# Hawkeye-FineGrained/Hawkeye

Hardware: NVIDIA H100
Metric: 448x448 images/sec, BCNN VGG-16 train step (fwd+CE+bwd+grad all-reduce+SGD), device-timed, max over ranks (higher is better)
Workload: dtype tf32 (fp32 storage, fp32 accumulate)

## Files before the change

### hawkeye_b200/csrc/common.cuh

```cuda
#pragma once
#include <cuda.h>
#include <cuda_runtime.h>
#include <stdint.h>
#include <stdio.h>

namespace hk {

#ifndef HK_SPIN_LIMIT
#define HK_SPIN_LIMIT (1u << 26)
#endif

__device__ __forceinline__ uint32_t smem_u32(const void* p) {
  return static_cast<uint32_t>(__cvta_generic_to_shared(p));
}

__device__ __forceinline__ void mbar_init(uint64_t* bar, uint32_t count) {
  asm volatile("mbarrier.init.shared::cta.b64 [%0], %1;" ::"r"(smem_u32(bar)), "r"(count));
}
__device__ __forceinline__ void fence_barrier_init() {
  asm volatile("fence.mbarrier_init.release.cluster;" ::: "memory");
}
__device__ __forceinline__ void fence_proxy_async() {
  asm volatile("fence.proxy.async.shared::cta;" ::: "memory");
}
__device__ __forceinline__ void mbar_expect_tx(uint64_t* bar, uint32_t bytes) {
  asm volatile("mbarrier.arrive.expect_tx.shared::cta.b64 _, [%0], %1;" ::"r"(smem_u32(bar)), "r"(bytes)
               : "memory");
}
__device__ __forceinline__ void mbar_arrive(uint64_t* bar) {
  asm volatile("mbarrier.arrive.shared::cta.b64 _, [%0];" ::"r"(smem_u32(bar)) : "memory");
}
__device__ __forceinline__ bool mbar_try_wait(uint64_t* bar, uint32_t parity) {
  uint32_t ok;
  asm volatile(
      "{\n"
      ".reg .pred p;\n"
      "mbarrier.try_wait.parity.shared::cta.b64 p, [%1], %2;\n"
      "selp.u32 %0, 1, 0, p;\n"
      "}\n"
      : "=r"(ok)
      : "r"(smem_u32(bar)), "r"(parity)
      : "memory");
  return ok != 0;
}
__device__ __forceinline__ void mbar_wait(uint64_t* bar, uint32_t parity) {
  uint32_t spins = 0;
  while (!mbar_try_wait(bar, parity)) {
    if (++spins > HK_SPIN_LIMIT) __trap();
  }
}
__device__ __forceinline__ void mbar_wait_unguarded(uint64_t* bar, uint32_t parity) {
  while (!mbar_try_wait(bar, parity)) {
  }
}

template <int N>
__device__ __forceinline__ void regs_dealloc() { asm volatile("setmaxnreg.dec.sync.aligned.u32 %0;" ::"n"(N)); }
template <int N>
__device__ __forceinline__ void regs_alloc() { asm volatile("setmaxnreg.inc.sync.aligned.u32 %0;" ::"n"(N)); }

__device__ __forceinline__ void tma_prefetch_desc(const CUtensorMap* m) {
  asm volatile("prefetch.tensormap [%0];" ::"l"(m) : "memory");
}
__device__ __forceinline__ void tma_load_2d(void* dst, const CUtensorMap* m, uint64_t* bar, int c0, int c1) {
  asm volatile(
      "cp.async.bulk.tensor.2d.shared::cluster.global.mbarrier::complete_tx::bytes [%0], [%1, {%3, %4}], [%2];" ::"r"(
          smem_u32(dst)),
      "l"(m), "r"(smem_u32(bar)), "r"(c0), "r"(c1)
      : "memory");
}
__device__ __forceinline__ void tma_load_3d(void* dst, const CUtensorMap* m, uint64_t* bar, int c0, int c1, int c2) {
  asm volatile(
      "cp.async.bulk.tensor.3d.shared::cluster.global.mbarrier::complete_tx::bytes [%0], [%1, {%3, %4, %5}], [%2];" ::
          "r"(smem_u32(dst)),
      "l"(m), "r"(smem_u32(bar)), "r"(c0), "r"(c1), "r"(c2)
      : "memory");
}
__device__ __forceinline__ void tma_load_4d(void* dst, const CUtensorMap* m, uint64_t* bar, int c0, int c1, int c2,
                                            int c3) {
  asm volatile(
      "cp.async.bulk.tensor.4d.shared::cluster.global.mbarrier::complete_tx::bytes [%0], [%1, {%3, %4, %5, %6}], "
      "[%2];" ::"r"(smem_u32(dst)),
      "l"(m), "r"(smem_u32(bar)), "r"(c0), "r"(c1), "r"(c2), "r"(c3)
      : "memory");
}

__device__ __forceinline__ void wgmma_fence() { asm volatile("wgmma.fence.sync.aligned;" ::: "memory"); }
__device__ __forceinline__ void wgmma_commit() { asm volatile("wgmma.commit_group.sync.aligned;" ::: "memory"); }
template <int N>
__device__ __forceinline__ void wgmma_wait() { asm volatile("wgmma.wait_group.sync.aligned %0;" ::"n"(N) : "memory"); }
template <int NACC>
__device__ __forceinline__ void wgmma_keep(float (&d)[NACC]) {
#pragma unroll
  for (int i = 0; i < NACC; ++i) asm volatile("" : "+f"(d[i])::"memory");
}
__device__ __forceinline__ void wgmma_tf32(float (&d)[8], uint64_t adesc, uint64_t bdesc, int scale_d) {
  asm volatile(
      "{\n"
      ".reg .pred p;\n"
      "setp.ne.b32 p, %10, 0;\n"
      "wgmma.mma_async.sync.aligned.m64n16k8.f32.tf32.tf32 "
      "{%0, %1, %2, %3, %4, %5, %6, %7}, %8, %9, p, 1, 1;\n"
      "}\n"
      : "+f"(d[0]), "+f"(d[1]), "+f"(d[2]), "+f"(d[3]), "+f"(d[4]), "+f"(d[5]), "+f"(d[6]), "+f"(d[7])
      : "l"(adesc), "l"(bdesc), "r"(scale_d));
}
__device__ __forceinline__ void wgmma_tf32(float (&d)[16], uint64_t adesc, uint64_t bdesc, int scale_d) {
  asm volatile(
      "{\n"
      ".reg .pred p;\n"
      "setp.ne.b32 p, %18, 0;\n"
      "wgmma.mma_async.sync.aligned.m64n32k8.f32.tf32.tf32 "
      "{%0, %1, %2, %3, %4, %5, %6, %7, %8, %9, %10, %11, %12, %13, %14, %15}, %16, %17, p, 1, 1;\n"
      "}\n"
      : "+f"(d[0]), "+f"(d[1]), "+f"(d[2]), "+f"(d[3]), "+f"(d[4]), "+f"(d[5]), "+f"(d[6]), "+f"(d[7]), "+f"(d[8]), "+f"(d[9]), "+f"(d[10]), "+f"(d[11]), "+f"(d[12]), "+f"(d[13]), "+f"(d[14]), "+f"(d[15])
      : "l"(adesc), "l"(bdesc), "r"(scale_d));
}
__device__ __forceinline__ void wgmma_tf32(float (&d)[32], uint64_t adesc, uint64_t bdesc, int scale_d) {
  asm volatile(
      "{\n"
      ".reg .pred p;\n"
      "setp.ne.b32 p, %34, 0;\n"
      "wgmma.mma_async.sync.aligned.m64n64k8.f32.tf32.tf32 "
      "{%0, %1, %2, %3, %4, %5, %6, %7, %8, %9, %10, %11, %12, %13, %14, %15, %16, %17, %18, %19, %20, %21, %22, %23, %24, %25, %26, %27, %28, %29, %30, %31}, %32, %33, p, 1, 1;\n"
      "}\n"
      : "+f"(d[0]), "+f"(d[1]), "+f"(d[2]), "+f"(d[3]), "+f"(d[4]), "+f"(d[5]), "+f"(d[6]), "+f"(d[7]), "+f"(d[8]), "+f"(d[9]), "+f"(d[10]), "+f"(d[11]), "+f"(d[12]), "+f"(d[13]), "+f"(d[14]), "+f"(d[15]), "+f"(d[16]), "+f"(d[17]), "+f"(d[18]), "+f"(d[19]), "+f"(d[20]), "+f"(d[21]), "+f"(d[22]), "+f"(d[23]), "+f"(d[24]), "+f"(d[25]), "+f"(d[26]), "+f"(d[27]), "+f"(d[28]), "+f"(d[29]), "+f"(d[30]), "+f"(d[31])
      : "l"(adesc), "l"(bdesc), "r"(scale_d));
}
__device__ __forceinline__ void wgmma_tf32(float (&d)[64], uint64_t adesc, uint64_t bdesc, int scale_d) {
  asm volatile(
      "{\n"
      ".reg .pred p;\n"
      "setp.ne.b32 p, %66, 0;\n"
      "wgmma.mma_async.sync.aligned.m64n128k8.f32.tf32.tf32 "
      "{%0, %1, %2, %3, %4, %5, %6, %7, %8, %9, %10, %11, %12, %13, %14, %15, %16, %17, %18, %19, %20, %21, %22, %23, %24, %25, %26, %27, %28, %29, %30, %31, %32, %33, %34, %35, %36, %37, %38, %39, %40, %41, %42, %43, %44, %45, %46, %47, %48, %49, %50, %51, %52, %53, %54, %55, %56, %57, %58, %59, %60, %61, %62, %63}, %64, %65, p, 1, 1;\n"
      "}\n"
      : "+f"(d[0]), "+f"(d[1]), "+f"(d[2]), "+f"(d[3]), "+f"(d[4]), "+f"(d[5]), "+f"(d[6]), "+f"(d[7]), "+f"(d[8]), "+f"(d[9]), "+f"(d[10]), "+f"(d[11]), "+f"(d[12]), "+f"(d[13]), "+f"(d[14]), "+f"(d[15]), "+f"(d[16]), "+f"(d[17]), "+f"(d[18]), "+f"(d[19]), "+f"(d[20]), "+f"(d[21]), "+f"(d[22]), "+f"(d[23]), "+f"(d[24]), "+f"(d[25]), "+f"(d[26]), "+f"(d[27]), "+f"(d[28]), "+f"(d[29]), "+f"(d[30]), "+f"(d[31]), "+f"(d[32]), "+f"(d[33]), "+f"(d[34]), "+f"(d[35]), "+f"(d[36]), "+f"(d[37]), "+f"(d[38]), "+f"(d[39]), "+f"(d[40]), "+f"(d[41]), "+f"(d[42]), "+f"(d[43]), "+f"(d[44]), "+f"(d[45]), "+f"(d[46]), "+f"(d[47]), "+f"(d[48]), "+f"(d[49]), "+f"(d[50]), "+f"(d[51]), "+f"(d[52]), "+f"(d[53]), "+f"(d[54]), "+f"(d[55]), "+f"(d[56]), "+f"(d[57]), "+f"(d[58]), "+f"(d[59]), "+f"(d[60]), "+f"(d[61]), "+f"(d[62]), "+f"(d[63])
      : "l"(adesc), "l"(bdesc), "r"(scale_d));
}

__device__ __forceinline__ void wgmma_tf32(float (&d)[8], const uint32_t (&a)[4], uint64_t bdesc) {
  asm volatile(
      "wgmma.mma_async.sync.aligned.m64n16k8.f32.tf32.tf32 "
      "{%0, %1, %2, %3, %4, %5, %6, %7}, {%8, %9, %10, %11}, %12, 1, 1, 1;\n"
      : "+f"(d[0]), "+f"(d[1]), "+f"(d[2]), "+f"(d[3]), "+f"(d[4]), "+f"(d[5]), "+f"(d[6]), "+f"(d[7])
      : "r"(a[0]), "r"(a[1]), "r"(a[2]), "r"(a[3]), "l"(bdesc));
}
__device__ __forceinline__ void wgmma_tf32(float (&d)[16], const uint32_t (&a)[4], uint64_t bdesc) {
  asm volatile(
      "wgmma.mma_async.sync.aligned.m64n32k8.f32.tf32.tf32 "
      "{%0, %1, %2, %3, %4, %5, %6, %7, %8, %9, %10, %11, %12, %13, %14, %15}, {%16, %17, %18, %19}, %20, 1, 1, 1;\n"
      : "+f"(d[0]), "+f"(d[1]), "+f"(d[2]), "+f"(d[3]), "+f"(d[4]), "+f"(d[5]), "+f"(d[6]), "+f"(d[7]), "+f"(d[8]), "+f"(d[9]), "+f"(d[10]), "+f"(d[11]), "+f"(d[12]), "+f"(d[13]), "+f"(d[14]), "+f"(d[15])
      : "r"(a[0]), "r"(a[1]), "r"(a[2]), "r"(a[3]), "l"(bdesc));
}
__device__ __forceinline__ void wgmma_tf32(float (&d)[32], const uint32_t (&a)[4], uint64_t bdesc) {
  asm volatile(
      "wgmma.mma_async.sync.aligned.m64n64k8.f32.tf32.tf32 "
      "{%0, %1, %2, %3, %4, %5, %6, %7, %8, %9, %10, %11, %12, %13, %14, %15, %16, %17, %18, %19, %20, %21, %22, %23, %24, %25, %26, %27, %28, %29, %30, %31}, {%32, %33, %34, %35}, %36, 1, 1, 1;\n"
      : "+f"(d[0]), "+f"(d[1]), "+f"(d[2]), "+f"(d[3]), "+f"(d[4]), "+f"(d[5]), "+f"(d[6]), "+f"(d[7]), "+f"(d[8]), "+f"(d[9]), "+f"(d[10]), "+f"(d[11]), "+f"(d[12]), "+f"(d[13]), "+f"(d[14]), "+f"(d[15]), "+f"(d[16]), "+f"(d[17]), "+f"(d[18]), "+f"(d[19]), "+f"(d[20]), "+f"(d[21]), "+f"(d[22]), "+f"(d[23]), "+f"(d[24]), "+f"(d[25]), "+f"(d[26]), "+f"(d[27]), "+f"(d[28]), "+f"(d[29]), "+f"(d[30]), "+f"(d[31])
      : "r"(a[0]), "r"(a[1]), "r"(a[2]), "r"(a[3]), "l"(bdesc));
}

__device__ __forceinline__ void named_bar(int id, int count) {
  asm volatile("bar.sync %0, %1;" ::"r"(id), "r"(count) : "memory");
}

__device__ __forceinline__ uint64_t make_sdesc(uint32_t saddr) {
  uint64_t d = 0;
  d |= static_cast<uint64_t>((saddr >> 4) & 0x3FFFu);
  d |= static_cast<uint64_t>(1) << 16;
  d |= static_cast<uint64_t>(1024 >> 4) << 32;
  d |= static_cast<uint64_t>(1) << 62;
  return d;
}

__device__ __forceinline__ uint32_t ld_shared_u32(uint32_t saddr) {
  uint32_t v;
  asm volatile("ld.shared.b32 %0, [%1];" : "=r"(v) : "r"(saddr) : "memory");
  return v;
}
__device__ __forceinline__ void st_shared_v4(uint32_t saddr, uint32_t x, uint32_t y, uint32_t z, uint32_t w) {
  asm volatile("st.shared.v4.b32 [%0], {%1, %2, %3, %4};" ::"r"(saddr), "r"(x), "r"(y), "r"(z), "r"(w) : "memory");
}

__device__ __forceinline__ uint32_t sw128_off(int row, int k) {
  return (uint32_t)(row * 128 + ((((k >> 2) ^ (row & 7)) << 4) | ((k & 3) << 2)));
}

__device__ __forceinline__ void transpose_mn_tile(const uint8_t* src, uint8_t* dst, int rows, int t, int nthr,
                                                  int box_stride = 4096) {
// ... 23 lines not shown
```

### hawkeye_b200/csrc/conv.cu

```cuda
#include <stdlib.h>

#include "common.cuh"
#include "host.h"
#include "gemm.h"
#include "../../include/hawkeye_b200.h"

namespace hk {

__global__ void pack_weights_kernel(const float* __restrict__ W, float* __restrict__ Wf, float* __restrict__ Wd,
                                    int Cout, int Cin, int round) {
  const size_t n = (size_t)Cout * Cin * 9;
  for (size_t i = blockIdx.x * (size_t)blockDim.x + threadIdx.x; i < n; i += (size_t)gridDim.x * blockDim.x) {
    const int t = i % 9;
    const int ci = (i / 9) % Cin;
    const int co = i / ((size_t)9 * Cin);
    const float v = round ? tf32_round(W[i]) : W[i];
    if (Wf) Wf[((size_t)t * Cout + co) * Cin + ci] = v;
    if (Wd) Wd[((size_t)(8 - t) * Cin + ci) * Cout + co] = v;
  }
}
__global__ void unpack_wgrad_kernel(const float* __restrict__ dWp, float* __restrict__ dW, int Cout, int Cin, int accumulate) {
  const size_t n = (size_t)Cout * Cin * 9;
  for (size_t i = blockIdx.x * (size_t)blockDim.x + threadIdx.x; i < n; i += (size_t)gridDim.x * blockDim.x) {
    const int t = i % 9;
// ... 114 lines not shown
    if (a.no_round) {
#pragma unroll
      for (int j = 0; j < 8; ++j) dst[j] = make_float4(v[4 * j], v[4 * j + 1], v[4 * j + 2], v[4 * j + 3]);
    } else {
#pragma unroll
      for (int j = 0; j < 8; ++j)
        dst[j] = make_float4(tf32_round(v[4 * j]), tf32_round(v[4 * j + 1]), tf32_round(v[4 * j + 2]),
                             tf32_round(v[4 * j + 3]));
    }
    }
  }
  if ((POOLED || a.P) && co < a.Cout) epi_pool_store(a, v, a.TW, w, h, n, co, valid);
}

template <int BN>
__device__ __forceinline__ void conv_epilogue(const ConvArgs& a, const float (&acc)[BN / 2], float* acc_tile, int w0, int h0,
                                              int n0, int co0, int ct) {
  constexpr int NACC = BN / 2;
  const int lane = ct & 31, wg = ct >> 7, half = ct >> 7;
  const int q = (ct >> 5) & 3, wl = q;
  const int r = q * 32 + lane;
  const int wi = r % a.TW, hi = (r / a.TW) % a.TH, ni = r / (a.TW * a.TH);
  const int w = w0 + wi, h = h0 + hi, n = n0 + ni;
  const bool valid = (w < a.W) && (h < a.H) && (n < a.N);
  const size_t pix = ((size_t)n * a.H + h) * a.W + w;
#pragma unroll
  for (int cp = 0; cp < BN / 64; ++cp) {
    named_bar(1, 256);
#pragma unroll
    for (int i = 0; i < NACC / 4; ++i) {
      const int col = 8 * i + 2 * (lane & 3);
      if ((col >> 6) != cp) continue;
      float* dst = acc_tile + ((col >> 5) & 1) * (128 * 33);
      const int r0 = wg * 64 + wl * 16 + (lane >> 2);
      dst[r0 * 33 + (col & 31)] = acc[4 * i];
      dst[r0 * 33 + (col & 31) + 1] = acc[4 * i + 1];
      dst[(r0 + 8) * 33 + (col & 31)] = acc[4 * i + 2];
      dst[(r0 + 8) * 33 + (col & 31) + 1] = acc[4 * i + 3];
    }
    named_bar(1, 256);
    const int c = 2 * cp + half;
    float v[32];
    {
      const float* src = acc_tile + half * (128 * 33) + r * 33;
#pragma unroll
      for (int j = 0; j < 32; ++j) v[j] = src[j];
    }
    epi_chunk(a, v, w, h, n, pix, co0 + c * 32, valid);
  }
}

template <int BN>
__global__ void __launch_bounds__(CONV_THREADS, 1)
conv3x3_igemm_kernel(const __grid_constant__ CUtensorMap tmX, const __grid_constant__ CUtensorMap tmW, ConvArgs a) {
  using Cfg = ConvCfg<BN>;
  constexpr int NACC = BN / 2;
  extern __shared__ uint8_t smem_raw[];
  uint8_t* smem = reinterpret_cast<uint8_t*>((reinterpret_cast<uintptr_t>(smem_raw) + 1023) & ~uintptr_t(1023));
  uint8_t* sA = smem;
  uint8_t* sB = smem + Cfg::STAGES * Cfg::A_BYTES;
  uint64_t* full = reinterpret_cast<uint64_t*>(smem + Cfg::STAGES * Cfg::STAGE_BYTES);
  uint64_t* empty = full + Cfg::STAGES;
  float* acc_tile = reinterpret_cast<float*>(smem + Cfg::STAGES * Cfg::STAGE_BYTES + 256);

  const int warp = threadIdx.x >> 5;
  int t = blockIdx.x;
  const int tw = t % a.tiles_w; t /= a.tiles_w;
  const int th = t % a.tiles_h; t /= a.tiles_h;
  const int w0 = tw * a.TW, h0 = th * a.TH, n0 = t * a.TN;
  const int co0 = blockIdx.y * BN;
  const int nchunk = a.Cin / 32;
  const int nk = 9 * nchunk;

  if (threadIdx.x == 0) {
    tma_prefetch_desc(&tmX);
    tma_prefetch_desc(&tmW);
    for (int s = 0; s < Cfg::STAGES; ++s) { mbar_init(&full[s], 1); mbar_init(&empty[s], 2); }
    fence_barrier_init();
  }
  __syncthreads();

  if (warp < 4) {
    regs_dealloc<56>();
    if (threadIdx.x == 0) {
      for (int kb = 0; kb < nk; ++kb) {
        const int s = kb % Cfg::STAGES;
        const uint32_t ph = (kb / Cfg::STAGES) & 1;
        const int tap = kb / nchunk, ck = kb - tap * nchunk;
        const int kh = tap / 3, kw = tap - kh * 3;
        mbar_wait(&empty[s], ph ^ 1);
        mbar_expect_tx(&full[s], Cfg::STAGE_BYTES);
        tma_load_4d(sA + s * Cfg::A_BYTES, &tmX, &full[s], ck * 32, w0 * a.stride + kw - 1, h0 * a.stride + kh - 1, n0);
        tma_load_3d(sB + s * Cfg::B_BYTES, &tmW, &full[s], ck * 32, co0, tap);
      }
    }
  } else {
    regs_alloc<224>();
    const int ct = threadIdx.x - 128;
    const int wg = ct >> 7;
    float acc[NACC];
    for (int kb = 0; kb < nk; ++kb) {
      const int s = kb % Cfg::STAGES;
      const uint32_t ph = (kb / Cfg::STAGES) & 1;
      mbar_wait(&full[s], ph);
      const uint64_t a_base = make_sdesc(smem_u32(sA + s * Cfg::A_BYTES + wg * 64 * 128));
      const uint64_t b_base = make_sdesc(smem_u32(sB + s * Cfg::B_BYTES));
      wgmma_fence();
#pragma unroll
      for (int ks = 0; ks < 4; ++ks) wgmma_tf32(acc, a_base + ks * 2, b_base + ks * 2, (kb | ks) != 0);
      wgmma_commit();
      wgmma_wait<1>();
      wgmma_keep(acc);
      if (kb > 0 && (ct & 127) == 0) mbar_arrive(&empty[(kb - 1) % Cfg::STAGES]);
    }
    wgmma_wait<0>();
    wgmma_keep(acc);
    conv_epilogue<BN>(a, acc, acc_tile, w0, h0, n0, co0, ct);
  }
}

static void pick_tile(int W, int H, int N, int target, int* TW, int* TH, int* TN) {
  int tw = 1;
  while (tw * 2 <= 16 && W % (tw * 2) == 0 && tw * 2 <= target) tw *= 2;
  int th = 1;
  while (th * 2 * tw <= target && H % (th * 2) == 0) th *= 2;
  int tn = target / (tw * th);
  *TW = tw; *TH = th; *TN = tn;
  (void)N;
}

static int make_act_map(CUtensorMap* tm, const float* X, int N, int H, int W, int C, int TW, int TH, int TN,
                        int stride = 1) {
  uint64_t dims[4] = {(uint64_t)C, (uint64_t)W, (uint64_t)H, (uint64_t)N};
  uint64_t strides[3] = {(uint64_t)C * 4, (uint64_t)W * C * 4, (uint64_t)H * W * C * 4};
  uint32_t box[4] = {32, (uint32_t)(TW * stride), (uint32_t)(TH * stride), (uint32_t)TN};
  uint32_t estr[4] = {1, (uint32_t)stride, (uint32_t)stride, 1};
  return make_tmap(tm, X, 4, dims, strides, box, stride > 1 ? estr : nullptr);
}

template <int BN>
static int launch_conv(const CUtensorMap& tmX, const CUtensorMap& tmW, const ConvArgs& a, cudaStream_t stream) {
  using Cfg = ConvCfg<BN>;
  if (int r = allow_dynamic_smem<conv3x3_igemm_kernel<BN>>(Cfg::SMEM, BN == 64 ? "conv<64>" : "conv<128>")) return r;
  dim3 grid(a.tiles_w * a.tiles_h * a.tiles_n, (a.Cout + BN - 1) / BN);
  conv3x3_igemm_kernel<BN><<<grid, CONV_THREADS, Cfg::SMEM, stream>>>(tmX, tmW, a);
  HK_LAUNCH_CHECK("conv3x3_igemm_kernel");
  return 0;
}

constexpr int CONV_V2_THREADS = 512;

enum { EPI_MAP = 0, EPI_UNPOOL = 1, EPI_FIRST_WGRAD = 2 };
constexpr int FW_HALO = 3 * 10 * 18;
constexpr int FW_HALO_BYTES = 2 * FW_HALO * 4;
struct FirstWgradArgs {
  const float* img;
  float* part;
};

__device__ __forceinline__ void mma_m16n8k8_tf32(float (&d)[4], const uint32_t (&a)[4], uint32_t b0, uint32_t b1) {
  asm volatile("mma.sync.aligned.m16n8k8.row.col.f32.tf32.tf32.f32 {%0, %1, %2, %3}, {%4, %5, %6, %7}, {%8, %9}, "
               "{%0, %1, %2, %3};\n"
               : "+f"(d[0]), "+f"(d[1]), "+f"(d[2]), "+f"(d[3])
               : "r"(a[0]), "r"(a[1]), "r"(a[2]), "r"(a[3]), "r"(b0), "r"(b1));
}

template <int BN, bool RESIDENT>
struct ConvV2Cfg {
  static constexpr int A_BYTES = 160 * 128;
  static constexpr int B_TILE = BN * 128;
  static constexpr int STAGE_BYTES = A_BYTES + (RESIDENT ? 0 : 3 * B_TILE);
  static constexpr int STAGES = RESIDENT ? 2 : (BN == 64 ? 3 : 2);
  static constexpr int WRES_BYTES = RESIDENT ? 18 * B_TILE : 0;
  static constexpr int PIECES = STAGES == 2 && !RESIDENT ? 3 : 1;
  static constexpr int STG_LD = BN + 8;
  static constexpr int STG_BYTES = 128 * STG_LD * 4;
  static constexpr int SMEM = STAGES * STAGE_BYTES + WRES_BYTES + 1024 + 256 + STG_BYTES;
};

template <int BN, bool RESIDENT, int TW, int EPI>
__global__ void __launch_bounds__(CONV_V2_THREADS, 1)
conv3x3_igemm_v2_kernel(const __grid_constant__ CUtensorMap tmX, const __grid_constant__ CUtensorMap tmW, ConvArgs a,
                        int n_ntiles, int total_tiles, FirstWgradArgs fw) {
  using Cfg = ConvV2Cfg<BN, RESIDENT>;
  static_assert(EPI != EPI_FIRST_WGRAD || (BN == 64 && RESIDENT && TW == 16), "conv1_1 weight gradient: 64 -> 64, 16 x 8");
  constexpr int NACC = BN / 2;
  constexpr int TN = 16 / TW;
  constexpr int WG_ROWS = TW == 16 ? 64 : 80;
  extern __shared__ uint8_t smem_raw[];
  uint8_t* smem = reinterpret_cast<uint8_t*>((reinterpret_cast<uintptr_t>(smem_raw) + 1023) & ~uintptr_t(1023));
  uint8_t* stages = smem;
  uint8_t* wres = smem + Cfg::STAGES * Cfg::STAGE_BYTES;
  uint64_t* full = reinterpret_cast<uint64_t*>(wres + Cfg::WRES_BYTES);
  uint64_t* empty = full + Cfg::STAGES * Cfg::PIECES;
  uint64_t* wbar = empty + Cfg::STAGES;
  uint64_t* stg_full = wbar + 1;
  uint64_t* stg_empty = wbar + 2;
  float* stg = reinterpret_cast<float*>(wres + Cfg::WRES_BYTES + 256);

  const int warp = threadIdx.x >> 5;
  const int nchunk = a.Cin / 32;
  const int nkb = nchunk * 3;

  if (threadIdx.x == 0) {
    tma_prefetch_desc(&tmX);
    tma_prefetch_desc(&tmW);
    for (int s = 0; s < Cfg::STAGES; ++s) mbar_init(&empty[s], 2);
    for (int i = 0; i < Cfg::STAGES * Cfg::PIECES; ++i) mbar_init(&full[i], 1);
    mbar_init(wbar, 1);
    mbar_init(stg_full, 256);
    mbar_init(stg_empty, 128);
    fence_barrier_init();
  }
  __syncthreads();

  if (warp >= 12 && EPI == EPI_MAP && a.P) {
    const int r = threadIdx.x - 384;
    int j = 0;
    for (int t = blockIdx.x; t < total_tiles; t += gridDim.x, ++j) {
      int pt = t / n_ntiles;
      const int co0 = (t - pt * n_ntiles) * BN;
      const int tw = pt % a.tiles_w; pt /= a.tiles_w;
      const int th = pt % a.tiles_h; pt /= a.tiles_h;
      mbar_wait(stg_full, j & 1);
      const int w = tw * TW + (r & (TW - 1)), h = th * 8 + ((r / TW) & 7), n = pt * TN + r / (TW * 8);
      const bool valid = TN == 1 || n < a.N;
      const size_t pix = ((size_t)n * a.H + h) * a.W + w;
#pragma unroll 1
      for (int c = 0; c < BN / 32; ++c) {
        float v[32];
        const float4* src = reinterpret_cast<const float4*>(stg + r * Cfg::STG_LD + c * 32);
#pragma unroll
        for (int k = 0; k < 8; ++k) {
          const float4 q = src[k];
          v[4 * k] = q.x; v[4 * k + 1] = q.y; v[4 * k + 2] = q.z; v[4 * k + 3] = q.w;
        }
        if (c == BN / 32 - 1) mbar_arrive(stg_empty);
        epi_chunk<true>(a, v, w, h, n, pix, co0 + c * 32, valid);
      }
    }
  } else if (warp >= 12) {
    const int e = threadIdx.x - 384;
    const int ew = e >> 5, sub = (e >> 3) & 3, u4 = (e & 7) * 4;
    const int p0 = ew * 32 + sub;
    const int eoff0 = (TW == 16 ? (p0 >> 4) * a.W + (p0 & 15) : ((p0 >> 6) * a.H + ((p0 >> 3) & 7)) * a.W + (p0 & 7)) * a.Cout + u4;
    const int erow = a.W * a.Cout, e4 = 4 * a.Cout;
    auto eoff = [&](int k) { return eoff0 + (k / (TW / 4)) * erow + (k % (TW / 4)) * e4; };
    const float* srow = stg + (ew * 32 + sub) * Cfg::STG_LD + u4;
    auto tile_org = [&](int t, size_t& org, int& co0) {
      co0 = (t % n_ntiles) * BN;
      int pt = t / n_ntiles;
      const int tw = pt % a.tiles_w; pt /= a.tiles_w;
      const int th = pt % a.tiles_h; pt /= a.tiles_h;
      org = (((size_t)pt * TN * a.H + th * 8) * a.W + tw * TW) * a.Cout;
      return pt * TN + (TW == 16 ? 0 : ew >> 1) < a.N;
    };
    auto tile_pos = [&](int t, int& tw, int& th, int& tn) {
      int pt = t / n_ntiles;
      tw = pt % a.tiles_w; pt /= a.tiles_w;
      th = pt % a.tiles_h; tn = pt / a.tiles_h;
    };
    const int frow = 2 * a.W * a.Cout;
    const int uoff0 = (TW == 16 ? 2 * (p0 >> 4) * frow + 2 * (p0 & 15) * a.Cout
                                : ((p0 >> 6) * 2 * a.H + 2 * ((p0 >> 3) & 7)) * frow + 2 * (p0 & 7) * a.Cout) + u4;
    auto uoff = [&](int k) { return uoff0 + (k / (TW / 4)) * 2 * frow + (k % (TW / 4)) * 8 * a.Cout; };
    float* halo = stg + 128 * Cfg::STG_LD;
    float dacc[4][4] = {};
    const int lane = e & 31, g = lane >> 2, tq = lane & 3;
    int hoff[4];
#pragma unroll
    for (int nt = 0; nt < 4; ++nt) {
      const int jj = 8 * nt + g;
      hoff[nt] = jj < 27 ? (jj / 9) * 180 + (jj % 9 / 3) * 18 + jj % 3 : 0;
    }
    int co0 = 0, j = 0;
    size_t org = 0;
    for (int t = blockIdx.x; t < total_tiles; t += gridDim.x, ++j) {
      const bool valid = tile_org(t, org, co0);
      if constexpr (EPI == EPI_FIRST_WGRAD) {
        int tw, th, tn;
        tile_pos(t, tw, th, tn);
        float* hb = halo + (j & 1) * FW_HALO;
        for (int i = e; i < FW_HALO; i += 128) {
          const int ci = i / 180, hh = th * 8 - 1 + i / 18 % 10, ww = tw * 16 - 1 + i % 18;
          hb[i] = hh >= 0 && hh < a.H && ww >= 0 && ww < a.W
                      ? tf32_round(__ldg(fw.img + (((size_t)tn * 3 + ci) * a.H + hh) * a.W + ww)) : 0.f;
        }
      }
      mbar_wait(stg_full, j & 1);
#pragma unroll
      for (int c = 0; c < BN / 32; ++c) {
        float4 v[8];
#pragma unroll
        for (int k = 0; k < 8; ++k) v[k] = *reinterpret_cast<const float4*>(srow + 4 * k * Cfg::STG_LD + c * 32);
        if (EPI != EPI_FIRST_WGRAD && c == BN / 32 - 1) mbar_arrive(stg_empty);
        const int co = co0 + c * 32;
        const bool live = valid && co < a.Cout;
        if (live) {
          if (a.bias) {
            const float4 b = __ldg(reinterpret_cast<const float4*>(a.bias + co + u4));
#pragma unroll
            for (int k = 0; k < 8; ++k) { v[k].x += b.x; v[k].y += b.y; v[k].z += b.z; v[k].w += b.w; }
          }
          if (a.relu) {
#pragma unroll
            for (int k = 0; k < 8; ++k) {
              v[k].x = fmaxf(v[k].x, 0.f); v[k].y = fmaxf(v[k].y, 0.f);
              v[k].z = fmaxf(v[k].z, 0.f); v[k].w = fmaxf(v[k].w, 0.f);
            }
          }
          if (a.mask) {
            float4 mk[8];
#pragma unroll
            for (int k = 0; k < 8; ++k) mk[k] = __ldcs(reinterpret_cast<const float4*>(a.mask + org + co + eoff(k)));
#pragma unroll
            for (int k = 0; k < 8; ++k) {
              v[k].x = mk[k].x > 0.f ? v[k].x : 0.f; v[k].y = mk[k].y > 0.f ? v[k].y : 0.f;
              v[k].z = mk[k].z > 0.f ? v[k].z : 0.f; v[k].w = mk[k].w > 0.f ? v[k].w : 0.f;
            }
          }
          if constexpr (EPI == EPI_MAP) {
#pragma unroll
            for (int k = 0; k < 8; ++k)
              __stcs(reinterpret_cast<float4*>(a.Y + org + co + eoff(k)),
                     make_float4(tf32_round(v[k].x), tf32_round(v[k].y), tf32_round(v[k].z), tf32_round(v[k].w)));
          } else if constexpr (EPI == EPI_UNPOOL) {
            int tw, th, tn;
            tile_pos(t, tw, th, tn);
            float* dst = a.Y + (((size_t)tn * TN * 2 * a.H + th * 16) * 2 * a.W + tw * 2 * TW) * a.Cout + co;
            uint32_t cd[8];
#pragma unroll
            for (int k = 0; k < 8; ++k) cd[k] = __ldcs(reinterpret_cast<const unsigned int*>(a.code + org + co + eoff(k)));
#pragma unroll
            for (int k = 0; k < 8; ++k) {
              const float4 q = make_float4((cd[k] & 4u) ? tf32_round(v[k].x) : 0.f, (cd[k] & (4u << 8)) ? tf32_round(v[k].y) : 0.f,
                                           (cd[k] & (4u << 16)) ? tf32_round(v[k].z) : 0.f,
                                           (cd[k] & (4u << 24)) ? tf32_round(v[k].w) : 0.f);
              float* o = dst + uoff(k);
#pragma unroll
              for (int pos = 0; pos < 4; ++pos)
                __stcs(reinterpret_cast<float4*>(o + (pos >> 1) * frow + (pos & 1) * a.Cout),
                       make_float4((cd[k] & 3u) == (uint32_t)pos ? q.x : 0.f, (cd[k] >> 8 & 3u) == (uint32_t)pos ? q.y : 0.f,
                                   (cd[k] >> 16 & 3u) == (uint32_t)pos ? q.z : 0.f,
                                   (cd[k] >> 24 & 3u) == (uint32_t)pos ? q.w : 0.f));
            }
          } else {
#pragma unroll
            for (int k = 0; k < 8; ++k)
              *reinterpret_cast<float4*>(stg + (ew * 32 + sub + 4 * k) * Cfg::STG_LD + u4 + c * 32) =
                  make_float4(tf32_round(v[k].x), tf32_round(v[k].y), tf32_round(v[k].z), tf32_round(v[k].w));
          }
        }
      }
      if constexpr (EPI == EPI_FIRST_WGRAD) {
        named_bar(1, 128);
        const float* hb = halo + (j & 1) * FW_HALO;
        const float* arow = stg + tq * Cfg::STG_LD + 16 * ew + g;
#pragma unroll 4
        for (int ks = 0; ks < 16; ++ks) {
          const float* ap = arow + 8 * ks * Cfg::STG_LD;
          const uint32_t af[4] = {__float_as_uint(ap[0]), __float_as_uint(ap[8]), __float_as_uint(ap[4 * Cfg::STG_LD]),
                                  __float_as_uint(ap[4 * Cfg::STG_LD + 8])};
          const int hp = (ks >> 1) * 18 + 8 * (ks & 1) + tq;
#pragma unroll
          for (int nt = 0; nt < 4; ++nt) {
            float b0 = hb[hoff[nt] + hp], b1 = hb[hoff[nt] + hp + 4];
            if (nt == 3 && g >= 3) b0 = b1 = g == 3 ? 1.f : 0.f;
            mma_m16n8k8_tf32(dacc[nt], af, __float_as_uint(b0), __float_as_uint(b1));
          }
        }
        mbar_arrive(stg_empty);
      }
    }
    if constexpr (EPI == EPI_FIRST_WGRAD) {
      float* dst = fw.part + (size_t)blockIdx.x * 64 * 32;
#pragma unroll
      for (int nt = 0; nt < 4; ++nt)
#pragma unroll
        for (int i = 0; i < 4; ++i) dst[(16 * ew + g + 8 * (i >> 1)) * 32 + 8 * nt + 2 * tq + (i & 1)] = dacc[nt][i];
    }
  } else if (warp < 4) {
    if (threadIdx.x == 0) {
      if (RESIDENT) {
        mbar_expect_tx(wbar, Cfg::WRES_BYTES);
        for (int tap = 0; tap < 9; ++tap)
          for (int ck = 0; ck < 2; ++ck) tma_load_3d(wres + (tap * 2 + ck) * Cfg::B_TILE, &tmW, wbar, ck * 32, 0, tap);
      }
      int kbg = 0;
      for (int t = blockIdx.x; t < total_tiles; t += gridDim.x) {
        const int nt = t % n_ntiles;
        int pt = t / n_ntiles;
        const int tw = pt % a.tiles_w; pt /= a.tiles_w;
        const int th = pt % a.tiles_h; pt /= a.tiles_h;
        const int w0 = tw * TW, h0 = th * 8, n0 = pt * TN, co0 = nt * BN;
        for (int kb = 0; kb < nkb; ++kb, ++kbg) {
          const int s = kbg % Cfg::STAGES;
          const uint32_t ph = (kbg / Cfg::STAGES) & 1;
          const int ck = kb / 3, kw = kb - ck * 3;
          mbar_wait(&empty[s], ph ^ 1);
          uint64_t* f = full + s * Cfg::PIECES;
          uint8_t* st = stages + s * Cfg::STAGE_BYTES;
          mbar_expect_tx(&f[0], Cfg::PIECES == 3 ? Cfg::A_BYTES + Cfg::B_TILE : Cfg::STAGE_BYTES);
          tma_load_4d(st, &tmX, &f[0], ck * 32, w0 + kw - 1, h0 - 1, n0);
          if (!RESIDENT) {
#pragma unroll
            for (int kh = 0; kh < 3; ++kh) {
              uint64_t* fk = &f[Cfg::PIECES == 3 ? kh : 0];
              if (Cfg::PIECES == 3 && kh > 0) mbar_expect_tx(fk, Cfg::B_TILE);
              tma_load_3d(st + Cfg::A_BYTES + kh * Cfg::B_TILE, &tmW, fk, ck * 32, co0, kh * 3 + kw);
            }
          }
        }
      }
    }
  } else {
    const int ct = threadIdx.x - 128;
    const int wg = ct >> 7;
    if (RESIDENT) mbar_wait(wbar, 0);
    float acc[NACC];
#pragma unroll
    for (int i = 0; i < NACC; ++i) acc[i] = 0.f;
    float* frag = stg + (wg * 64 + ((ct >> 5) & 3) * 16 + ((ct & 31) >> 2)) * Cfg::STG_LD + 2 * (ct & 3);
    int kbg = 0, j = 0;
    for (int t = blockIdx.x; t < total_tiles; t += gridDim.x, ++j) {
      for (int kb = 0; kb < nkb; ++kb, ++kbg) {
        const int s = kbg % Cfg::STAGES;
        const int ck = kb / 3, kw = kb - ck * 3;
        const uint32_t ph = (kbg / Cfg::STAGES) & 1;
        const uint32_t a_addr = smem_u32(stages + s * Cfg::STAGE_BYTES) + wg * WG_ROWS * 128;
#pragma unroll
        for (int kh = 0; kh < 3; ++kh) {
          if (kh < Cfg::PIECES) {
            mbar_wait(&full[s * Cfg::PIECES + kh], ph);
            wgmma_fence();
          }
          const uint32_t b_addr = RESIDENT ? smem_u32(wres + ((kh * 3 + kw) * 2 + ck) * Cfg::B_TILE)
                                           : smem_u32(stages + s * Cfg::STAGE_BYTES + Cfg::A_BYTES + kh * Cfg::B_TILE);
          const uint64_t ad = make_sdesc(a_addr + kh * TW * 128), bd = make_sdesc(b_addr);
#pragma unroll
          for (int ks = 0; ks < 4; ++ks) wgmma_tf32(acc, ad + ks * 2, bd + ks * 2, (kb | kh | ks) != 0);
          if (kh >= 3 - Cfg::PIECES) wgmma_commit();
          if (kh == 3 - Cfg::PIECES) {
            wgmma_wait<1>();
            wgmma_keep(acc);
            if (kb > 0 && (ct & 127) == 0) mbar_arrive(&empty[(kbg - 1) % Cfg::STAGES]);
          }
        }
      }
      wgmma_wait<0>();
      wgmma_keep(acc);
      if ((ct & 127) == 0) mbar_arrive(&empty[(kbg - 1) % Cfg::STAGES]);
      mbar_wait(stg_empty, (j & 1) ^ 1);
#pragma unroll
      for (int i = 0; i < NACC / 4; ++i) {
        *reinterpret_cast<float2*>(frag + 8 * i) = make_float2(acc[4 * i], acc[4 * i + 1]);
        *reinterpret_cast<float2*>(frag + 8 * Cfg::STG_LD + 8 * i) = make_float2(acc[4 * i + 2], acc[4 * i + 3]);
      }
      mbar_arrive(stg_full);
    }
  }
}

template <int BN, bool RESIDENT, int TW, int EPI = EPI_MAP>
static int launch_conv_v2(const float* x, const float* wp, ConvArgs a, int N, int H, int W, cudaStream_t stream,
                          FirstWgradArgs fw = {}) {
  using Cfg = ConvV2Cfg<BN, RESIDENT>;
  constexpr int SMEM = Cfg::SMEM + (EPI == EPI_FIRST_WGRAD ? FW_HALO_BYTES : 0);
  static_assert(SMEM <= 232448, "conv_v2: dynamic shared memory above the sm_90 opt-in limit");
  if (int r = allow_dynamic_smem<conv3x3_igemm_v2_kernel<BN, RESIDENT, TW, EPI>>(SMEM, BN == 64 ? "conv_v2<64>" : "conv_v2<128>"))
    return r;
  a.TW = TW; a.TH = 8; a.TN = 16 / TW;
  a.tiles_w = W / TW; a.tiles_h = H / 8; a.tiles_n = (N + a.TN - 1) / a.TN;
  const int n_ntiles = (a.Cout + BN - 1) / BN;
  const long long total = (long long)a.tiles_w * a.tiles_h * a.tiles_n * n_ntiles;
  HK_REQUIRE(total < (1ll << 31), HK_ERR_UNSUPPORTED, "conv3x3: too many tiles");
  HK_REQUIRE((long long)H * W * a.Cout < (1ll << 30), HK_ERR_UNSUPPORTED, "conv3x3: map too large");
  CUtensorMap tmX, tmW;
  int r;
  {
    uint64_t dims[4] = {(uint64_t)a.Cin, (uint64_t)W, (uint64_t)H, (uint64_t)N};
    uint64_t strides[3] = {(uint64_t)a.Cin * 4, (uint64_t)W * a.Cin * 4, (uint64_t)H * W * a.Cin * 4};
    uint32_t box[4] = {32, (uint32_t)TW, 10, (uint32_t)a.TN};
    if ((r = make_tmap(&tmX, x, 4, dims, strides, box))) return r;
  }
  {
    uint64_t dims[3] = {(uint64_t)a.Cin, (uint64_t)a.Cout, 9};
    uint64_t strides[2] = {(uint64_t)a.Cin * 4, (uint64_t)a.Cin * a.Cout * 4};
    uint32_t box[3] = {32, (uint32_t)BN, 1};
    if ((r = make_tmap(&tmW, wp, 3, dims, strides, box))) return r;
  }
  const int sms = num_sms();
  const int grid = total < sms ? (int)total : sms;
  conv3x3_igemm_v2_kernel<BN, RESIDENT, TW, EPI><<<grid, CONV_V2_THREADS, SMEM, stream>>>(tmX, tmW, a, n_ntiles, (int)total, fw);
  HK_LAUNCH_CHECK("conv3x3_igemm_v2_kernel");
  return 0;
}

template <int TW, int EPI = EPI_MAP>
static int launch_conv_v2(const float* x, const float* wp, const ConvArgs& a, int N, int H, int W, cudaStream_t stream) {
  if (a.Cin == 64 && a.Cout == 64) return launch_conv_v2<64, true, TW, EPI>(x, wp, a, N, H, W, stream);
  if (a.Cout <= 64) return launch_conv_v2<64, false, TW, EPI>(x, wp, a, N, H, W, stream);
  return launch_conv_v2<128, false, TW, EPI>(x, wp, a, N, H, W, stream);
}

static int conv3x3_igemm_1x(const float* x, const float* wp, const float* bias, const float* mask, const float* addend,
                            float* y, int N, int H, int W, int Cin, int Cout, int relu, cudaStream_t stream, int stride,
                            int no_round, float* pooled = nullptr, unsigned char* code = nullptr,
                            int pool_nchw = 0);

int conv3x3_igemm(const float* x, const float* wp, const float* bias, const float* mask, float* y, int N, int H, int W,
                  int Cin, int Cout, int relu, cudaStream_t stream, int stride = 1) {
  if (!precise()) return conv3x3_igemm_1x(x, wp, bias, mask, nullptr, y, N, H, W, Cin, Cout, relu, stream, stride, 0);
  HK_REQUIRE(x && wp && y, HK_ERR_ARG, "conv3x3: null pointer");
  const size_t nx = (size_t)N * H * W * Cin, nw = (size_t)9 * Cout * Cin;
  Scratch sx(2 * nx * sizeof(float), stream), sw(2 * nw * sizeof(float), stream);
  HK_REQUIRE(sx.p && sw.p, HK_ERR_DRIVER, "conv3x3 (precise): cudaMallocAsync of the operand halves failed");
  float *xh = sx.f(), *xl = xh + nx, *wh = sw.f(), *wl = wh + nw;
  int r;
  if ((r = tf32_split(x, xh, xl, nx, stream))) return r;
  if ((r = tf32_split(wp, wh, wl, nw, stream))) return r;
  if ((r = conv3x3_igemm_1x(xh, wl, nullptr, nullptr, nullptr, y, N, H, W, Cin, Cout, 0, stream, stride, 1))) return r;
  if ((r = conv3x3_igemm_1x(xl, wh, nullptr, nullptr, y, y, N, H, W, Cin, Cout, 0, stream, stride, 1))) return r;
  return conv3x3_igemm_1x(xh, wh, bias, mask, y, y, N, H, W, Cin, Cout, relu, stream, stride, 1);
}

static int conv3x3_igemm_1x(const float* x, const float* wp, const float* bias, const float* mask, const float* addend,
                            float* y, int N, int H, int W, int Cin, int Cout, int relu, cudaStream_t stream, int stride,
                            int no_round, float* pooled, unsigned char* code, int pool_nchw) {
  const int Hin = H, Win = W;
  if (stride == 2) {
    HK_REQUIRE(H % 2 == 0 && W % 2 == 0, HK_ERR_UNSUPPORTED, "conv3x3 stride 2: even H/W required");
    H /= 2; W /= 2;
  }
  HK_REQUIRE(x && wp && (y || pooled), HK_ERR_ARG, "conv3x3: null pointer");
  HK_REQUIRE(Cin % 32 == 0 && Cout % 32 == 0, HK_ERR_UNSUPPORTED, "conv3x3: Cin=%d Cout=%d must be multiples of 32",
             Cin, Cout);
  HK_REQUIRE(aligned16(x) && aligned16(wp) && (!y || aligned16(y)) && (!mask || aligned16(mask)), HK_ERR_ALIGN,
             "conv3x3: pointer not 16-byte aligned");
  if (pooled)
    HK_REQUIRE(stride == 1 && H % 2 == 0 && W % 2 == 0 && aligned16(pooled) && (!code || aligned16(code)), HK_ERR_UNSUPPORTED,
               "conv3x3 + pool: even H/W, stride 1 and 16-byte aligned outputs required");
  ConvArgs a = {};
  a.P = pooled; a.code = code; a.pool_nchw = pool_nchw;
  a.Y = y; a.bias = bias; a.mask = mask; a.N = N; a.H = H; a.W = W; a.Cin = Cin; a.Cout = Cout; a.relu = relu;
  a.stride = stride;
  a.addend = addend; a.no_round = no_round;
  if (!no_round && stride == 1 && W % 8 == 0 && H % 8 == 0) {
    if (W % 16 == 0) return launch_conv_v2<16>(x, wp, a, N, H, W, stream);
    return launch_conv_v2<8>(x, wp, a, N, H, W, stream);
  }
  pick_tile(W, H, N, 128, &a.TW, &a.TH, &a.TN);
  HK_REQUIRE(!pooled || (a.TW >= 2 && a.TH >= 2), HK_ERR_UNSUPPORTED, "conv3x3 + pool: pixel tile %dx%d", a.TW, a.TH);
  a.tiles_w = (W + a.TW - 1) / a.TW; a.tiles_h = (H + a.TH - 1) / a.TH; a.tiles_n = (N + a.TN - 1) / a.TN;
  HK_REQUIRE((long long)a.tiles_w * a.tiles_h * a.tiles_n < (1ll << 31), HK_ERR_UNSUPPORTED, "conv3x3: grid too large");
  CUtensorMap tmX, tmW;
  int r;
  if ((r = make_act_map(&tmX, x, N, Hin, Win, Cin, a.TW, a.TH, a.TN, stride))) return r;
  const int BN = Cout <= 64 ? 64 : 128;
  {
    uint64_t dims[3] = {(uint64_t)Cin, (uint64_t)Cout, 9};
    uint64_t strides[2] = {(uint64_t)Cin * 4, (uint64_t)Cin * Cout * 4};
    uint32_t box[3] = {32, (uint32_t)BN, 1};
    if ((r = make_tmap(&tmW, wp, 3, dims, strides, box))) return r;
  }
  if (BN == 64) return launch_conv<64>(tmX, tmW, a, stream);
  return launch_conv<128>(tmX, tmW, a, stream);
}

struct WgradArgs {
  float* dWp;
  float* db;
  int N, H, W, Cin, Cout;
  int TW, TH, TN, tiles_w, tiles_h, tiles_n;
  int total_tiles, per;
};

constexpr int WG_THREADS = 4 * 128;
constexpr int WG_PRODUCER_REGS = 56, WG_CONSUMER_REGS = 152;
static_assert(128 * WG_PRODUCER_REGS + 3 * 128 * WG_CONSUMER_REGS <= 65536, "wgrad register budget");
constexpr int WG_STAGES = 3;
constexpr int WG_KP = 64;
constexpr int WG_RAW_ROWS = 120;
constexpr int WG_RAW_BYTES = WG_RAW_ROWS * 128;

constexpr int WG_CI = 64, WG_CO = 64;
constexpr int WG_X_BYTES = (WG_CI / 32) * WG_RAW_BYTES;
constexpr int WG_DY_BYTES = (WG_CO / 32) * WG_KP * 128;
constexpr int WG_STAGE_BYTES = WG_X_BYTES + 2 * WG_DY_BYTES;
constexpr int WG_SMEM = WG_STAGES * WG_STAGE_BYTES + 1024 + 256;
static_assert(WG_SMEM <= 227 * 1024, "wgrad shared memory");

template <int TW, int TH, int TN>
struct WgradTile {
  int w0, h0, n0;
  __device__ __forceinline__ WgradTile(int t, const WgradArgs& a) {
    w0 = t % a.tiles_w * TW; t /= a.tiles_w;
    h0 = t % a.tiles_h * TH;
    n0 = t / a.tiles_h * TN;
  }
  __device__ __forceinline__ void next(const WgradArgs& a) {
    if ((w0 += TW) < a.W) return;
    w0 = 0;
    if ((h0 += TH) < a.H) return;
    h0 = 0;
    n0 += TN;
  }
};

template <int TW, int TH, int TN>
__global__ void __launch_bounds__(WG_THREADS, 1)
conv3x3_wgrad_kernel(const __grid_constant__ CUtensorMap tmDY, const __grid_constant__ CUtensorMap tmX, WgradArgs a) {
  static_assert(TW * TH * TN == WG_KP && TW % 8 == 0, "64-pixel tile of whole 8-pixel rows");
  static_assert((TH + 2) * (TW + 2) * TN <= WG_RAW_ROWS, "halo patch too large");
  extern __shared__ uint8_t smem_raw[];
  uint8_t* smem = reinterpret_cast<uint8_t*>((reinterpret_cast<uintptr_t>(smem_raw) + 1023) & ~uintptr_t(1023));
  uint64_t* full = reinterpret_cast<uint64_t*>(smem + WG_STAGES * WG_STAGE_BYTES);
  uint64_t* empty = full + WG_STAGES;
  uint64_t* dy_full = empty + WG_STAGES;
  const uint32_t stage0 = smem_u32(smem);

// ... 788 lines not shown
```

Baseline: 815.7.

## Split resident-weight conv epilogue staging into slices and add a third input stage

For resident-weight conv kernels (excluding the first-layer weight-gradient variant), the staging buffer now holds a 32-channel slice instead of the whole BN tile. The freed shared memory funds a third activation pipeline stage. The MMA warpgroups hand off the first slice at tile end and hold the second slice in registers. They push it opportunistically with a non-blocking mbarrier test_wait during the next tile's K loop, so the epilogue overlaps with the main loop. This adds register pressure from the held slice, more barrier phase traffic, and per-k-block polling overhead.

Result: no change. 819.7, median of 6 (+0.5%).

```diff
diff --git a/hawkeye_b200/csrc/common.cuh b/hawkeye_b200/csrc/common.cuh
--- a/hawkeye_b200/csrc/common.cuh
+++ b/hawkeye_b200/csrc/common.cuh
@@ -36,6 +36,19 @@
       "{\n"
       ".reg .pred p;\n"
       "mbarrier.try_wait.parity.shared::cta.b64 p, [%1], %2;\n"
+      "selp.u32 %0, 1, 0, p;\n"
+      "}\n"
+      : "=r"(ok)
+      : "r"(smem_u32(bar)), "r"(parity)
+      : "memory");
+  return ok != 0;
+}
+__device__ __forceinline__ bool mbar_test_wait(uint64_t* bar, uint32_t parity) {
+  uint32_t ok;
+  asm volatile(
+      "{\n"
+      ".reg .pred p;\n"
+      "mbarrier.test_wait.parity.shared::cta.b64 p, [%1], %2;\n"
       "selp.u32 %0, 1, 0, p;\n"
       "}\n"
       : "=r"(ok)
diff --git a/hawkeye_b200/csrc/conv.cu b/hawkeye_b200/csrc/conv.cu
--- a/hawkeye_b200/csrc/conv.cu
+++ b/hawkeye_b200/csrc/conv.cu
@@ -290,7 +290,6 @@
 
 enum { EPI_MAP = 0, EPI_UNPOOL = 1, EPI_FIRST_WGRAD = 2 };
 constexpr int FW_HALO = 3 * 10 * 18;
-constexpr int FW_HALO_BYTES = 2 * FW_HALO * 4;
 struct FirstWgradArgs {
   const float* img;
   float* part;
@@ -303,26 +302,32 @@
                : "r"(a[0]), "r"(a[1]), "r"(a[2]), "r"(a[3]), "r"(b0), "r"(b1));
 }
 
-template <int BN, bool RESIDENT>
+template <int BN, bool RESIDENT, int EPI>
 struct ConvV2Cfg {
   static constexpr int A_BYTES = 160 * 128;
   static constexpr int B_TILE = BN * 128;
   static constexpr int STAGE_BYTES = A_BYTES + (RESIDENT ? 0 : 3 * B_TILE);
-  static constexpr int STAGES = RESIDENT ? 2 : (BN == 64 ? 3 : 2);
+  static constexpr int STAGES = RESIDENT ? (EPI == EPI_FIRST_WGRAD ? 2 : 3) : (BN == 64 ? 3 : 2);
   static constexpr int WRES_BYTES = RESIDENT ? 18 * B_TILE : 0;
   static constexpr int PIECES = STAGES == 2 && !RESIDENT ? 3 : 1;
-  static constexpr int STG_LD = BN + 8;
+  static constexpr int SLICE = RESIDENT && EPI != EPI_FIRST_WGRAD ? 32 : BN;
+  static constexpr int NSLICE = BN / SLICE;
+  static constexpr int STG_LD = SLICE + 8;
   static constexpr int STG_BYTES = 128 * STG_LD * 4;
-  static constexpr int SMEM = STAGES * STAGE_BYTES + WRES_BYTES + 1024 + 256 + STG_BYTES;
+  static constexpr int HALO_BYTES = EPI == EPI_FIRST_WGRAD ? 2 * FW_HALO * 4 : 0;
+  static constexpr int SMEM = STAGES * STAGE_BYTES + WRES_BYTES + 1024 + 256 + STG_BYTES + HALO_BYTES;
+  static_assert(SMEM <= 232448, "conv_v2: dynamic shared memory above the sm_90 opt-in limit");
+  static_assert(NSLICE <= 2, "the MMA warpgroups hold back at most one slice of a finished tile");
 };
 
 template <int BN, bool RESIDENT, int TW, int EPI>
 __global__ void __launch_bounds__(CONV_V2_THREADS, 1)
 conv3x3_igemm_v2_kernel(const __grid_constant__ CUtensorMap tmX, const __grid_constant__ CUtensorMap tmW, ConvArgs a,
                         int n_ntiles, int total_tiles, FirstWgradArgs fw) {
-  using Cfg = ConvV2Cfg<BN, RESIDENT>;
+  using Cfg = ConvV2Cfg<BN, RESIDENT, EPI>;
   static_assert(EPI != EPI_FIRST_WGRAD || (BN == 64 && RESIDENT && TW == 16), "conv1_1 weight gradient: 64 -> 64, 16 x 8");
   constexpr int NACC = BN / 2;
+  constexpr int CPS = Cfg::SLICE / 32;
   constexpr int TN = 16 / TW;
   constexpr int WG_ROWS = TW == 16 ? 64 : 80;
   extern __shared__ uint8_t smem_raw[];
@@ -354,26 +359,30 @@
 
   if (warp >= 12 && EPI == EPI_MAP && a.P) {
     const int r = threadIdx.x - 384;
-    int j = 0;
-    for (int t = blockIdx.x; t < total_tiles; t += gridDim.x, ++j) {
+    uint32_t hs = 0;
+    for (int t = blockIdx.x; t < total_tiles; t += gridDim.x) {
       int pt = t / n_ntiles;
       const int co0 = (t - pt * n_ntiles) * BN;
       const int tw = pt % a.tiles_w; pt /= a.tiles_w;
       const int th = pt % a.tiles_h; pt /= a.tiles_h;
-      mbar_wait(stg_full, j & 1);
       const int w = tw * TW + (r & (TW - 1)), h = th * 8 + ((r / TW) & 7), n = pt * TN + r / (TW * 8);
       const bool valid = TN == 1 || n < a.N;
       const size_t pix = ((size_t)n * a.H + h) * a.W + w;
 #pragma unroll 1
       for (int c = 0; c < BN / 32; ++c) {
+        const int cc = c % CPS;
+        if (cc == 0) mbar_wait(stg_full, hs & 1);
         float v[32];
-        const float4* src = reinterpret_cast<const float4*>(stg + r * Cfg::STG_LD + c * 32);
+        const float4* src = reinterpret_cast<const float4*>(stg + r * Cfg::STG_LD + cc * 32);
 #pragma unroll
         for (int k = 0; k < 8; ++k) {
           const float4 q = src[k];
           v[4 * k] = q.x; v[4 * k + 1] = q.y; v[4 * k + 2] = q.z; v[4 * k + 3] = q.w;
         }
-        if (c == BN / 32 - 1) mbar_arrive(stg_empty);
+        if (cc == CPS - 1) {
+          mbar_arrive(stg_empty);
+          ++hs;
+        }
         epi_chunk<true>(a, v, w, h, n, pix, co0 + c * 32, valid);
       }
     }
@@ -402,6 +411,7 @@
     const int uoff0 = (TW == 16 ? 2 * (p0 >> 4) * frow + 2 * (p0 & 15) * a.Cout
                                 : ((p0 >> 6) * 2 * a.H + 2 * ((p0 >> 3) & 7)) * frow + 2 * (p0 & 7) * a.Cout) + u4;
     auto uoff = [&](int k) { return uoff0 + (k / (TW / 4)) * 2 * frow + (k % (TW / 4)) * 8 * a.Cout; };
+    static_assert(EPI != EPI_FIRST_WGRAD || Cfg::NSLICE == 1, "conv1_1 weight gradient: the whole tile in one hand-off");
     float* halo = stg + 128 * Cfg::STG_LD;
     float dacc[4][4] = {};
     const int lane = e & 31, g = lane >> 2, tq = lane & 3;
@@ -411,27 +421,32 @@
       const int jj = 8 * nt + g;
       hoff[nt] = jj < 27 ? (jj / 9) * 180 + (jj % 9 / 3) * 18 + jj % 3 : 0;
     }
-    int co0 = 0, j = 0;
+    int co0 = 0;
+    uint32_t hs = 0;
     size_t org = 0;
-    for (int t = blockIdx.x; t < total_tiles; t += gridDim.x, ++j) {
+    for (int t = blockIdx.x; t < total_tiles; t += gridDim.x) {
       const bool valid = tile_org(t, org, co0);
       if constexpr (EPI == EPI_FIRST_WGRAD) {
         int tw, th, tn;
         tile_pos(t, tw, th, tn);
-        float* hb = halo + (j & 1) * FW_HALO;
+        float* hb = halo + (hs & 1) * FW_HALO;
         for (int i = e; i < FW_HALO; i += 128) {
           const int ci = i / 180, hh = th * 8 - 1 + i / 18 % 10, ww = tw * 16 - 1 + i % 18;
           hb[i] = hh >= 0 && hh < a.H && ww >= 0 && ww < a.W
                       ? tf32_round(__ldg(fw.img + (((size_t)tn * 3 + ci) * a.H + hh) * a.W + ww)) : 0.f;
         }
       }
-      mbar_wait(stg_full, j & 1);
 #pragma unroll
       for (int c = 0; c < BN / 32; ++c) {
+        const int cc = c % CPS;
+        if (cc == 0) mbar_wait(stg_full, hs & 1);
         float4 v[8];
 #pragma unroll
-        for (int k = 0; k < 8; ++k) v[k] = *reinterpret_cast<const float4*>(srow + 4 * k * Cfg::STG_LD + c * 32);
-        if (EPI != EPI_FIRST_WGRAD && c == BN / 32 - 1) mbar_arrive(stg_empty);
+        for (int k = 0; k < 8; ++k) v[k] = *reinterpret_cast<const float4*>(srow + 4 * k * Cfg::STG_LD + cc * 32);
+        if (EPI != EPI_FIRST_WGRAD && cc == CPS - 1) {
+          mbar_arrive(stg_empty);
+          ++hs;
+        }
         const int co = co0 + c * 32;
         const bool live = valid && co < a.Cout;
         if (live) {
@@ -485,14 +500,14 @@
           } else {
 #pragma unroll
             for (int k = 0; k < 8; ++k)
-              *reinterpret_cast<float4*>(stg + (ew * 32 + sub + 4 * k) * Cfg::STG_LD + u4 + c * 32) =
+              *reinterpret_cast<float4*>(stg + (ew * 32 + sub + 4 * k) * Cfg::STG_LD + u4 + cc * 32) =
                   make_float4(tf32_round(v[k].x), tf32_round(v[k].y), tf32_round(v[k].z), tf32_round(v[k].w));
           }
         }
       }
       if constexpr (EPI == EPI_FIRST_WGRAD) {
         named_bar(1, 128);
-        const float* hb = halo + (j & 1) * FW_HALO;
+        const float* hb = halo + (hs & 1) * FW_HALO;
         const float* arow = stg + tq * Cfg::STG_LD + 16 * ew + g;
 #pragma unroll 4
         for (int ks = 0; ks < 16; ++ks) {
@@ -508,6 +523,7 @@
           }
         }
         mbar_arrive(stg_empty);
+        ++hs;
       }
     }
     if constexpr (EPI == EPI_FIRST_WGRAD) {
@@ -558,9 +574,20 @@
     float acc[NACC];
 #pragma unroll
     for (int i = 0; i < NACC; ++i) acc[i] = 0.f;
+    constexpr int SL_ACC = NACC / Cfg::NSLICE;
     float* frag = stg + (wg * 64 + ((ct >> 5) & 3) * 16 + ((ct & 31) >> 2)) * Cfg::STG_LD + 2 * (ct & 3);
-    int kbg = 0, j = 0;
-    for (int t = blockIdx.x; t < total_tiles; t += gridDim.x, ++j) {
+    auto put_slice = [&](const float* v) {
+#pragma unroll
+      for (int i = 0; i < SL_ACC / 4; ++i) {
+        *reinterpret_cast<float2*>(frag + 8 * i) = make_float2(v[4 * i], v[4 * i + 1]);
+        *reinterpret_cast<float2*>(frag + 8 * Cfg::STG_LD + 8 * i) = make_float2(v[4 * i + 2], v[4 * i + 3]);
+      }
+    };
+    float held[Cfg::NSLICE > 1 ? SL_ACC : 1];
+    bool holding = false;
+    uint32_t hs = 0;
+    int kbg = 0;
+    for (int t = blockIdx.x; t < total_tiles; t += gridDim.x) {
       for (int kb = 0; kb < nkb; ++kb, ++kbg) {
         const int s = kbg % Cfg::STAGES;
         const int ck = kb / 3, kw = kb - ck * 3;
@@ -584,16 +611,37 @@
             if (kb > 0 && (ct & 127) == 0) mbar_arrive(&empty[(kbg - 1) % Cfg::STAGES]);
           }
         }
+        if constexpr (Cfg::NSLICE > 1) {
+          if (holding && __shfl_sync(0xffffffffu, (int)mbar_test_wait(stg_empty, (hs & 1) ^ 1), 0)) {
+            put_slice(held);
+            mbar_arrive(stg_full);
+            ++hs;
+            holding = false;
+          }
+        }
       }
       wgmma_wait<0>();
       wgmma_keep(acc);
       if ((ct & 127) == 0) mbar_arrive(&empty[(kbg - 1) % Cfg::STAGES]);
-      mbar_wait(stg_empty, (j & 1) ^ 1);
-#pragma unroll
-      for (int i = 0; i < NACC / 4; ++i) {
-        *reinterpret_cast<float2*>(frag + 8 * i) = make_float2(acc[4 * i], acc[4 * i + 1]);
-        *reinterpret_cast<float2*>(frag + 8 * Cfg::STG_LD + 8 * i) = make_float2(acc[4 * i + 2], acc[4 * i + 3]);
-      }
+      if (Cfg::NSLICE > 1 && holding) {
+        mbar_wait(stg_empty, (hs & 1) ^ 1);
+        put_slice(held);
+        mbar_arrive(stg_full);
+        ++hs;
+      }
+      mbar_wait(stg_empty, (hs & 1) ^ 1);
+      put_slice(acc);
+      mbar_arrive(stg_full);
+      ++hs;
+      if constexpr (Cfg::NSLICE > 1) {
+#pragma unroll
+        for (int i = 0; i < SL_ACC; ++i) held[i] = acc[SL_ACC + i];
+        holding = true;
+      }
+    }
+    if (Cfg::NSLICE > 1 && holding) {
+      mbar_wait(stg_empty, (hs & 1) ^ 1);
+      put_slice(held);
       mbar_arrive(stg_full);
     }
   }
@@ -602,8 +650,7 @@
 template <int BN, bool RESIDENT, int TW, int EPI = EPI_MAP>
 static int launch_conv_v2(const float* x, const float* wp, ConvArgs a, int N, int H, int W, cudaStream_t stream,
                           FirstWgradArgs fw = {}) {
-  using Cfg = ConvV2Cfg<BN, RESIDENT>;
-  constexpr int SMEM = Cfg::SMEM + (EPI == EPI_FIRST_WGRAD ? FW_HALO_BYTES : 0);
+  constexpr int SMEM = ConvV2Cfg<BN, RESIDENT, EPI>::SMEM;
   static_assert(SMEM <= 232448, "conv_v2: dynamic shared memory above the sm_90 opt-in limit");
   if (int r = allow_dynamic_smem<conv3x3_igemm_v2_kernel<BN, RESIDENT, TW, EPI>>(SMEM, BN == 64 ? "conv_v2<64>" : "conv_v2<128>"))
     return r;
```
